# hanyujin02/trajectory_planner

Hardware: AMD Instinct MI355X
Metric: B-spline trajs/s (32 ctrl pts, 256^3 grid, 50 iters) @1 GPU; % HBM roofline (higher is better)
Workload: dtype f64

## Files before the change

trajectory_planner_amd/csrc/vigo_solver.hip:

```cpp
#include <stdlib.h>

#include <type_traits>

#include "vigo_internal.hpp"

namespace vigo {
namespace {

constexpr int kWave = 64;
constexpr int kMaxMem = VIGO_MAX_MEM_SIZE;
constexpr int kObsTabObs = 16;
template <int GROUP> constexpr int kObsTabEntries = GROUP == 32 ? 88 : 33;
template <int GROUP> constexpr int kObsTabDoubles = 3 * kObsTabEntries<GROUP> + kObsTabObs;

enum : int {
    LB_CONVERGENCE = 0,
    LB_STOP = 1,
    LB_ALREADY_MINIMIZED = 2,
    LBERR_UNKNOWN = -1024,
    LBERR_LOGIC,
    LBERR_CANCELED,
    LBERR_INVALID_N,
    LBERR_INVALID_MEMSIZE,
    LBERR_INVALID_GEPSILON,
// ... 56 lines not shown
__device__ __forceinline__ double dpp_f64(double v) {
    const int lo = __builtin_amdgcn_mov_dpp(__double2loint(v), CTRL, 0xF, 0xF, false);
    const int hi = __builtin_amdgcn_mov_dpp(__double2hiint(v), CTRL, 0xF, 0xF, false);
    return __hiloint2double(hi, lo);
}
__device__ __forceinline__ double add_f64_again(double a, double b) {
    double r;
    asm volatile("v_add_f64 %0, %1, %2" : "=v"(r) : "v"(a), "v"(b));
    return r;
}
__device__ __forceinline__ void xor16_parts(double a, double b, double& p0, double& p1) {
    const int alo = __double2loint(a), ahi = __double2hiint(a), blo = __double2loint(b), bhi = __double2hiint(b);
    auto l = __builtin_amdgcn_permlane16_swap(alo, blo, false, false);
    auto h = __builtin_amdgcn_permlane16_swap(ahi, bhi, false, false);
    p0 = __hiloint2double(h[0], l[0]);
    p1 = __hiloint2double(h[1], l[1]);
}
__device__ __forceinline__ double xor32_sum2(double a, double b) {
    const int alo = __double2loint(a), ahi = __double2hiint(a), blo = __double2loint(b), bhi = __double2hiint(b);
    auto l = __builtin_amdgcn_permlane32_swap(alo, blo, false, false);
    auto h = __builtin_amdgcn_permlane32_swap(ahi, bhi, false, false);
    return __hiloint2double(h[0], l[0]) + __hiloint2double(h[1], l[1]);
}
template <int GROUP, int K>
__device__ __forceinline__ void group_sum(double (&v)[K]) {
    static_assert(GROUP == 16 || GROUP == 32 || GROUP == 64, "group is a DPP row, half a wave or a wave");
#pragma unroll
    for (int q = 0; q < K; ++q) v[q] += dpp_f64<0xB1>(v[q]);
#pragma unroll
    for (int q = 0; q < K; ++q) v[q] += dpp_f64<0x4E>(v[q]);
#pragma unroll
    for (int q = 0; q < K; ++q) v[q] += dpp_f64<0x141>(v[q]);
    if (GROUP >= 32) {
#pragma unroll
        for (int q = 0; q < K; ++q) {
            const double t = dpp_f64<0x140>(v[q]);
            const double a = v[q] + t;
            const double b = add_f64_again(v[q], t);
            double p0, p1;
            xor16_parts(a, b, p0, p1);
            if (GROUP == 64) v[q] = xor32_sum2(p0 + p1, add_f64_again(p0, p1));
            else v[q] = p0 + p1;
        }
        return;
    }
#pragma unroll
// ... 29 lines not shown
        auto l2 = __builtin_amdgcn_permlane32_swap(xlo, xlo, false, false);
        auto h2 = __builtin_amdgcn_permlane32_swap(xhi, xhi, false, false);
        mx = fmax(__hiloint2double(h2[0], l2[0]), __hiloint2double(h2[1], l2[1]));
    }
}

__device__ __forceinline__ double sum3(double a, double b, double c) { return (a + b) + c; }

__device__ __forceinline__ double fmaT(double a, double b, double c) { return __builtin_fma(a, b, c); }
__device__ __forceinline__ float fmaT(float a, float b, float c) { return __builtin_fmaf(a, b, c); }

template <bool FAST, typename T, int D = 3>
__device__ __forceinline__ double dot3(const T (&a)[3], const T (&b)[3]) {
    if (D == 2) {
        if (FAST) return fmaT((double)a[1], (double)b[1], (double)a[0] * (double)b[0]);
        return (double)a[0] * (double)b[0] + (double)a[1] * (double)b[1];
    }
    if (FAST)
        return fmaT((double)a[2], (double)b[2], fmaT((double)a[1], (double)b[1], (double)a[0] * (double)b[0]));
    return sum3((double)a[0] * (double)b[0], (double)a[1] * (double)b[1], (double)a[2] * (double)b[2]);
}
template <bool FAST, typename T, int PPL, int D = 3>
__device__ __forceinline__ double dot_lane(const T (&a)[PPL][3], const T (&b)[PPL][3]) {
    double s = dot3<FAST, T, D>(a[0], b[0]);
#pragma unroll
    for (int q = 1; q < PPL; ++q) s += dot3<FAST, T, D>(a[q], b[q]);
    return s;
}

template <bool FAST>
struct YSv {
    double v, r;
};
template <>
struct YSv<true> {
    double v;
};
__device__ __forceinline__ bool exp_in_safe_range(double a) {
    const unsigned e = ((unsigned)__double2hiint(a) >> 20) & 0x7ffu;
    return (e - 523u) < 1000u;
}
__device__ __forceinline__ YSv<true> make_ys(double ys, YSv<true>*) { return YSv<true>{1.0 / ys}; }
__device__ __forceinline__ YSv<false> make_ys(double ys, YSv<false>*) {
    return YSv<false>{ys, exp_in_safe_range(ys) ? 1.0 / ys : __builtin_nan("")};
}
template <bool MARK>
__device__ __forceinline__ double over_ys(double a, const YSv<true>& y, double&, double&) { return a * y.v; }
template <bool MARK>
__device__ __forceinline__ double over_ys(double a, const YSv<false>& y, double& amin, double& amax) {
    if (!MARK) return a / y.v;
// ... 12 lines not shown

template <typename T, int PPL>
struct LaneProblem {
    static constexpr int kGuideRegs = (PPL == 1) ? 2 : 0;
    static constexpr int kGuideDim = kGuideRegs > 0 ? kGuideRegs : 1;
    int N;
    bool level;
    int p0;
    bool has_pt[PPL];
    bool interior[PPL];
    int g_begin[PPL], g_end[PPL];
    const double* gpv;
    const uint8_t* gunk;
    T gq[kGuideDim][6];
    bool gqu[kGuideDim];
    int o_begin, o_end;
    const double* obs;
    const double* obs_tab;
    const double* obs_size;
    int o_tab, o_steps;
    double w[4];
};

template <bool FAST, typename T>
__device__ __forceinline__ void guide_pair_term(const DevConst& K, const T (&c)[3], T px, T py, T pz, T vx,
                                                T vy, T vz, bool unk, double& cd, T (&Gd)[3]) {
    const T dth = (T)K.dth, da = (T)K.da, db = (T)K.db, dcc = (T)K.dc, uf = (T)K.unc_factor;
    const T dist = FAST ? fmaT(c[2] - pz, vz, fmaT(c[1] - py, vy, (c[0] - px) * vx))
                        : ((c[0] - px) * vx + (c[1] - py) * vy) + (c[2] - pz) * vz;
    const T e = dth - dist;
    T ct, k;
    bool scale = false;
    if (e <= -dth) {
        const T ne = -e;
        ct = (ne * ne) * ne;
        k = T(3.0) * (ne * ne);
    } else if (e > T(0) && e <= dth) {
        ct = (e * e) * e;
        k = T(-3.0) * (e * e);
        scale = unk;
    } else if (e >= dth) {
        ct = (da * (e * e) + db * e) + dcc;
        k = -((T(2) * da) * e + db);
        scale = unk;
    } else {
        return;
    }
    T gx = k * vx, gy = k * vy, gz = k * vz;
    if (scale) { ct *= uf; gx *= uf; gy *= uf; gz *= uf; }
    if (!K.plan_in_z) gz = T(0.0);
    cd += (double)ct;
    Gd[0] += gx; Gd[1] += gy; Gd[2] += gz;
}

template <typename T>
__device__ __forceinline__ void obstacle_term(const DevConst& K, const T (&c)[3], T opx, T opy, T ovx, T ovy, T size,
                                              double& co, T (&Go)[3]) {
    const T thr0 = (T)K.thr_dyn, oa = (T)K.oa, ob = (T)K.ob, oc = (T)K.oc;
    for (int n = 0; n <= K.pred_num; n += 2) {
        const T tn = (T)((double)n * K.ts);
        const T px = opx + tn * ovx, py = opy + tn * ovy;
        const T thr = (T(1) - (T)(n / K.pred_num) * T(0.2)) * thr0;
        const T dx = c[0] - px, dy = c[1] - py, dz = T(0.0);
        const T nrm = sqrt((dx * dx + dy * dy) + dz * dz);
        const T e = thr - (nrm - size);
        if (e > T(0)) {
            const bool cubic = e <= thr;
            const T ct = cubic ? (e * e) * e : (oa * (e * e) + ob * e) + oc;
            const T k = cubic ? T(-3.0) * (e * e) : -((T(2) * oa) * e + ob);
            co += (double)ct;
            Go[0] += k * (dx / nrm); Go[1] += k * (dy / nrm);
            if (__builtin_expect(!(nrm > T(0) && nrm < (T)INFINITY), 0)) Go[2] += k * (dz / nrm);
        }
    }
}

template <typename T>
__device__ __forceinline__ void obstacle_term_tab(const DevConst& K, const T (&c)[3], const double* tab, int steps,
                                                  T size, double& co, T (&Go)[3]) {
    const T oa = (T)K.oa, ob = (T)K.ob, oc = (T)K.oc;
    for (int s = 0; s < steps; ++s) {
        const T px = (T)tab[3 * s + 0], py = (T)tab[3 * s + 1], thr = (T)tab[3 * s + 2];
        const T dx = c[0] - px, dy = c[1] - py, dz = T(0.0);
        const T nrm = sqrt((dx * dx + dy * dy) + dz * dz);
        const T e = thr - (nrm - size);
        if (e > T(0)) {
            const bool cubic = e <= thr;
            const T ct = cubic ? (e * e) * e : (oa * (e * e) + ob * e) + oc;
            const T k = cubic ? T(-3.0) * (e * e) : -((T(2) * oa) * e + ob);
            co += (double)ct;
            Go[0] += k * (dx / nrm); Go[1] += k * (dy / nrm);
            if (__builtin_expect(!(nrm > T(0) && nrm < (T)INFINITY), 0)) Go[2] += k * (dz / nrm);
        }
    }
}

template <typename T, int GROUP, int PPL, bool FAST, bool OBS = true, int D = 3>
__device__ __forceinline__ double eval_cost_grad(const DevConst& K, const LaneProblem<T, PPL>& Q,
                                                 const T (&c)[PPL][3], const T (&d)[PPL][3], T (&g)[PPL][3],
                                                 double (&sums)[7]) {
    using LP = LaneProblem<T, PPL>;
    const int N = Q.N;
    T Gd[PPL][3], Gs[PPL][3], Gf[PPL][3], Go[PPL][3];
    double pt_s[PPL], pt_f[PPL], pt_d[PPL], pt_o[PPL];
#pragma unroll
    for (int q = 0; q < PPL; ++q) {
        pt_s[q] = pt_f[q] = pt_d[q] = pt_o[q] = 0.0;
#pragma unroll
        for (int a = 0; a < 3; ++a) Gd[q][a] = Go[q][a] = T(0);
    }

    {
        const T ts = (T)K.ts_ctrl, tis = (T)K.ts_inv_sqr;
        auto excess = [](T v) -> T { return v > T(1.0) ? v - T(1.0) : (v < T(-1.0) ? v + T(1.0) : T(0.0)); };
        double jj[PPL][3], vv[PPL][3], aa[PPL][3];
#pragma unroll
        for (int a = 0; a < 3; ++a) {
            if (a >= D) {
#pragma unroll
                for (int q = 0; q < PPL; ++q) { jj[q][a] = vv[q][a] = aa[q][a] = 0.0; Gs[q][a] = Gf[q][a] = T(0); }
                continue;
            }
            T C[PPL], P1[PPL], P2[PPL], P3[PPL];
#pragma unroll
            for (int q = 0; q < PPL; ++q) C[q] = c[q][a];
            seq_next<T, PPL>(C, P1);
            seq_next<T, PPL>(P1, P2);
            seq_next<T, PPL>(P2, P3);
            T gt0[PPL], gv[PPL], ga[PPL];
#pragma unroll
            for (int q = 0; q < PPL; ++q) {
                T J0 = FAST ? fmaT(T(3), P1[q], fmaT(T(-3), P2[q], P3[q])) - C[q]
                            : ((P3[q] - 3 * P2[q]) + 3 * P1[q]) - C[q];
                if (a == 2 && Q.level) J0 = T(0);
                gt0[q] = T(2.0) * J0;
                jj[q][a] = (double)(J0 * J0);
                T evP = excess((P1[q] - C[q]) / ts);
                T eaP = excess((FAST ? fmaT(T(-2), P1[q], P2[q]) + C[q]
                                     : (P2[q] - 2 * P1[q]) + C[q]) * tis);
                if (a == 2 && Q.level) { evP = T(0); eaP = T(0); }
                gv[q] = (T(2) * evP) / ts * tis;
                ga[q] = (T(2) * eaP) * tis;
                vv[q][a] = (double)((evP * evP) * tis);
                aa[q][a] = (double)(eaP * eaP);
            }
            T gt1[PPL], gt2[PPL], gt3[PPL], gvM[PPL], gaM1[PPL], gaM2[PPL];
            seq_prev<T, PPL>(gt0, gt1);
            seq_prev<T, PPL>(gt1, gt2);
            seq_prev<T, PPL>(gt2, gt3);
            seq_prev<T, PPL>(gv, gvM);
            seq_prev<T, PPL>(ga, gaM1);
            seq_prev<T, PPL>(gaM1, gaM2);
#pragma unroll
            for (int q = 0; q < PPL; ++q) {
                T acc = gt3[q];
                if (FAST) {
                    acc = fmaT(T(-3.0), gt2[q], acc);
                    acc = fmaT(T(3.0), gt1[q], acc);
                } else {
                    acc += T(-3.0) * gt2[q];
                    acc += T(3.0) * gt1[q];
                }
                acc += -gt0[q];
                Gs[q][a] = acc;
                T fcc = gvM[q];
                fcc += -gv[q];
                fcc += gaM2[q];
                fcc += -(T(2) * gaM1[q]);
                fcc += ga[q];
                Gf[q][a] = fcc;
            }
        }
#pragma unroll
        for (int q = 0; q < PPL; ++q) {
            const int p = Q.p0 + q;
            if (Q.has_pt[q] && p <= N - 4) pt_s[q] = sum3(jj[q][0], jj[q][1], jj[q][2]);
            double cf = 0.0;
            if (Q.has_pt[q] && p <= N - 2) cf = (vv[q][0] + vv[q][1]) + vv[q][2];
            if (Q.has_pt[q] && p <= N - 3) { cf += aa[q][0]; cf += aa[q][1]; cf += aa[q][2]; }
            pt_f[q] = cf;
        }
    }

#pragma unroll
    for (int q = 0; q < PPL; ++q) {
        if (Q.interior[q]) {
            double cd = 0.0;
            const int cnt = Q.g_end[q] - Q.g_begin[q];
#pragma unroll
            for (int j = 0; j < LP::kGuideRegs; ++j) {
                if (j < cnt)
                    guide_pair_term<FAST, T>(K, c[q], Q.gq[j][0], Q.gq[j][1], Q.gq[j][2], Q.gq[j][3], Q.gq[j][4], Q.gq[j][5],
                                       Q.gqu[j], cd, Gd[q]);
            }
// ... 56 lines not shown
        const double v4 = dot3<FAST, T, D>(g[q], d[q]);
        const double v5 = Q.interior[q] ? dot3<FAST, T>(c[q], c[q]) : 0.0;
        const double v6 = dot3<FAST, T, D>(g[q], g[q]);
        if (q == 0) {
            part[0] = pt_d[0]; part[1] = pt_s[0]; part[2] = pt_f[0]; part[3] = pt_o[0];
            part[4] = v4; part[5] = v5; part[6] = v6;
        } else {
            part[0] += pt_d[q]; part[1] += pt_s[q]; part[2] += pt_f[q]; part[3] += pt_o[q];
            part[4] += v4; part[5] += v5; part[6] += v6;
        }
    }
    if (OBS) {
        group_sum<GROUP, 7>(part);
    } else {
        double p6[6] = {part[0], part[1], part[2], part[4], part[5], part[6]};
        group_sum<GROUP, 6>(p6);
        part[0] = p6[0]; part[1] = p6[1]; part[2] = p6[2]; part[3] = 0.0; part[4] = p6[3]; part[5] = p6[4]; part[6] = p6[5];
    }
#pragma unroll
    for (int q = 0; q < 7; ++q) sums[q] = part[q];
    return ((Q.w[0] * part[0] + Q.w[1] * part[1]) + Q.w[2] * part[2]) + Q.w[3] * part[3];
}

template <typename T, int GROUP, int PPL>
__device__ __forceinline__ void load_problem(const SolveArgs& A, const DevConst& K, int b, int lane_in_group,
                                             LaneProblem<T, PPL>& Q) {
    using LP = LaneProblem<T, PPL>;
    const int N = A.N;
    Q.N = N;
    Q.level = false;
    Q.p0 = lane_in_group * PPL;
    Q.gpv = A.guide_pv;
    Q.gunk = A.guide_unk;
#pragma unroll
    for (int q = 0; q < PPL; ++q) {
        const int p = Q.p0 + q;
        Q.has_pt[q] = p < N;
        Q.interior[q] = (p >= 3) && (p <= N - 4);
        Q.g_begin[q] = Q.g_end[q] = 0;
        if (Q.interior[q] && A.guide_off && A.guide_pv) {
            Q.g_begin[q] = A.guide_off[(size_t)b * N + p];
            Q.g_end[q] = A.guide_off[(size_t)b * N + p + 1];
        }
    }
#pragma unroll
    for (int j = 0; j < LP::kGuideDim; ++j) {
// ... 40 lines not shown
    }
}

template <typename T, int GROUP, int PPL>
__device__ __forceinline__ void set_level(const DevConst& K, LaneProblem<T, PPL>& Q, const T (&x)[PPL][3]) {
    double mn = INFINITY, mx = -INFINITY;
#pragma unroll
    for (int q = 0; q < PPL; ++q) {
        if (Q.has_pt[q]) { mn = fmin(mn, (double)x[q][2]); mx = fmax(mx, (double)x[q][2]); }
    }
    group_minmax<GROUP>(mn, mx);
    Q.level = !K.plan_in_z && !K.strict_z && (mx - mn) <= 0x1p-40 * fmax(1.0, fmax(fabs(mn), fabs(mx)));
}

template <typename T, int PPL>
__device__ __forceinline__ void store_points(const SolveArgs& A, int b, const LaneProblem<T, PPL>& Q, const T (&x)[PPL][3]) {
#pragma unroll
    for (int q = 0; q < PPL; ++q) {
        if (Q.has_pt[q]) {
            double* dst = A.ctrl + ((size_t)b * A.N + Q.p0 + q) * 3;
            dst[0] = (double)x[q][0]; dst[1] = (double)x[q][1]; dst[2] = (double)x[q][2];
        }
    }
}

template <typename T, int GROUP, int PPL, bool FAST>
__global__ void __launch_bounds__(kWave) k_cost_grad(SolveArgs A, const DevConst* __restrict__ Kp) {
    const DevConst& K = *Kp;
    constexpr int TPB = kWave / GROUP;
    const int lane = threadIdx.x;
    const int b = blockIdx.x * TPB + lane / GROUP;
    if (b >= A.B) return;
    LaneProblem<T, PPL> Q;
    load_problem<T, GROUP, PPL>(A, K, b, lane % GROUP, Q);
    T c[PPL][3], g[PPL][3], zero[PPL][3];
    load_points<T, PPL>(A, b, Q, c);
    set_level<T, GROUP, PPL>(K, Q, c);
#pragma unroll
    for (int q = 0; q < PPL; ++q) zero[q][0] = zero[q][1] = zero[q][2] = T(0);
    double sums[7];
    const double f = eval_cost_grad<T, GROUP, PPL, FAST>(K, Q, c, zero, g, sums);
#pragma unroll
    for (int q = 0; q < PPL; ++q) {
        if (Q.interior[q] && A.out_grad) {
            double* dst = A.out_grad + ((size_t)b * (A.N - 6) + (Q.p0 + q - 3)) * 3;
            dst[0] = (double)g[q][0]; dst[1] = (double)g[q][1]; dst[2] = (double)g[q][2];
// ... 109 lines not shown
    tt = newt;
    return 0;
}

#ifndef VIGO_PROFILE_SECTIONS
#define VIGO_PROFILE_SECTIONS 0
#endif
#if VIGO_PROFILE_SECTIONS
#define VIGO_TICK(acc)                                                   \
    do {                                                                 \
        __builtin_amdgcn_sched_barrier(0);                               \
        const long long now_ = (long long)__builtin_readcyclecounter();  \
        __builtin_amdgcn_sched_barrier(0);                               \
        acc += (double)(now_ - tick_);                                   \
        tick_ = now_;                                                    \
    } while (0)
#else
#define VIGO_TICK(acc) do { } while (0)
#endif

template <typename T, int GROUP, int PPL, bool FAST, int WPS = 1, bool OBS = true, int D = 3, int RH = (PPL == 1 ? 1 : 0)>
__global__ void __launch_bounds__(kWave, WPS) k_optimize(SolveArgs A, const DevConst* __restrict__ Kp) {
    static_assert(PPL == 1 ? (RH >= 1 && RH <= 6) : RH == 0, "register-held history only with one point per lane");
    const DevConst& K = *Kp;
    constexpr int TPB = kWave / GROUP;
    extern __shared__ __align__(16) unsigned char lds_raw[];
    const int N = A.N, NI = N - 6;
    const int ROW = TPB * NI;
    const int ROWP = ROW + 1;
    using YS = YSv<FAST>;
    constexpr int kYsSlotBytes = (TPB * (int)sizeof(YS) + 15) & ~15;
    const int slotB = ROWP * (int)sizeof(HPair<T, D>) + kYsSlotBytes;
    const int m = K.mem_size;
    constexpr bool REG1 = (PPL == 1);
    const int ms = REG1 ? (m > RH + 1 ? m - (RH + 1) : 0) : m;
    HPair<T, D>* hist = reinterpret_cast<HPair<T, D>*>(lds_raw);
    double* ys_tab = reinterpret_cast<double*>(lds_raw + (size_t)ms * slotB);

    const int lane = threadIdx.x;
    const int grp = lane / GROUP;
    int b = blockIdx.x * TPB + grp;
    if (A.active_idx) {
        if (b >= *A.active_count) return;
        b = A.active_idx[b];
    } else if (b >= A.B) {
        return;
    }

    LaneProblem<T, PPL> Q;
    load_problem<T, GROUP, PPL>(A, K, b, lane % GROUP, Q);
    T x[PPL][3];
    load_points<T, PPL>(A, b, Q, x);
    set_level<T, GROUP, PPL>(K, Q, x);
    {
        const bool wave_level = __all(Q.level);
        if (D == 2 && !wave_level) return;
        if (D == 3 && A.level_waves_elsewhere && wave_level) return;
    }
#if VIGO_PROFILE_SECTIONS
    long long tick_ = (long long)__builtin_readcyclecounter();
    double t_eval = 0, t_ls = 0, t_upd = 0, t_two = 0, t_tail = 0, t_pre = 0, t_trial = 0, t_cal = 0;
#endif
    HPair<T, D>* hl[PPL];
#pragma unroll
    for (int q = 0; q < PPL; ++q) {
        const int p = Q.p0 + q;
        hl[q] = Q.interior[q] ? hist + (grp * NI + (p - 3)) : hist + ROW;
    }
    for (int slot = lane; slot < ms; slot += kWave) {
        HPair<T, D> zero;
#pragma unroll
        for (int a = 0; a < D; ++a) zero.s[a] = zero.y[a] = T(0);
        *reinterpret_cast<HPair<T, D>*>(lds_raw + (size_t)slot * slotB + (size_t)ROW * sizeof(HPair<T, D>)) = zero;
    }
    __syncthreads();
    YS* ys_l = reinterpret_cast<YS*>(lds_raw + (size_t)ROWP * sizeof(HPair<T, D>)) + grp;
    double* al_l = ys_tab + grp;
    auto hist_at = [&](int q, int slot) -> HPair<T, D>& {
        return *reinterpret_cast<HPair<T, D>*>(reinterpret_cast<char*>(hl[q]) + (size_t)slot * slotB);
    };
    auto ys_at = [&](int slot) -> YS& { return *reinterpret_cast<YS*>(reinterpret_cast<char*>(ys_l) + (size_t)slot * slotB); };
    if (!OBS) { Q.obs = nullptr; Q.o_begin = Q.o_end = 0; }
    if (OBS && A.obs) {
        constexpr int kEnt = kObsTabEntries<GROUP>;
        double* tab = ys_tab + (size_t)m * TPB + (size_t)grp * kObsTabDoubles<GROUP>;
        const int cnt = Q.o_end - Q.o_begin;
        const int steps = K.pred_num / 2 + 1;
        int fit = kEnt / steps;
        if (fit > kObsTabObs) fit = kObsTabObs;
        Q.o_tab = cnt < fit ? cnt : fit;
        Q.o_steps = steps;
        Q.obs_tab = tab;
        Q.obs_size = tab + 3 * kEnt;
        for (int e = lane % GROUP; e < Q.o_tab * steps; e += GROUP) {
            const int j = e / steps, n = 2 * (e - j * steps);
            const double* o = A.obs + 9 * (size_t)(Q.o_begin + j);
            const T tn = (T)((double)n * K.ts);
            tab[3 * e + 0] = (double)((T)o[0] + tn * (T)o[3]);
            tab[3 * e + 1] = (double)((T)o[1] + tn * (T)o[4]);
            tab[3 * e + 2] = (double)((T(1) - (T)(n / K.pred_num) * T(0.2)) * (T)K.thr_dyn);
        }
        for (int j = lane % GROUP; j < Q.o_tab; j += GROUP) {
            const double* o = A.obs + 9 * (size_t)(Q.o_begin + j);
            const T hx = (T)o[6] / 2, hy = (T)o[7] / 2;
            tab[3 * kEnt + j] = (double)(T)sqrt(hx * hx + hy * hy);
        }
        __syncthreads();
    }

    T g[PPL][3], xp[PPL][3], gp[PPL][3], d[PPL][3];
#pragma unroll
    for (int q = 0; q < PPL; ++q)
#pragma unroll
        for (int a = 0; a < 3; ++a) g[q][a] = xp[q][a] = gp[q][a] = d[q][a] = T(0);
    constexpr int kRH = RH > 0 ? RH : 1;
    T sR[kRH][PPL][3], yR[kRH][PPL][3];
    YS ysR[kRH]{};
#pragma unroll
    for (int q = 0; q < PPL; ++q)
#pragma unroll
        for (int a = 0; a < 3; ++a)
#pragma unroll
            for (int j = 0; j < kRH; ++j) sR[j][q][a] = yR[j][q][a] = T(0);
    double sums[7];
    int evals = 0;
    int ret = LBERR_UNKNOWN;
    int k = 0, end = 0, last = 0;
    double fx = 0.0, step = 0.0;
    bool first = true;

    for (;;) {
        int ls = 0;
        int count = 0, brackt = 0, stage1 = 1, uinfo = 0;
        double dginit = 0.0, finit = 0.0, dgtest = 0.0, width = 0.0, prev_width = 0.0;
        double xt = 0., xf = 0., xd = 0., yt = 0., yf = 0., yd = 0.;
        const double stpmin = K.min_step, stpmax = K.max_step;
        bool run = true;
        if (!first) {
#pragma unroll
            for (int q = 0; q < PPL; ++q)
#pragma unroll
                for (int a = 0; a < D; ++a) { xp[q][a] = x[q][a]; gp[q][a] = g[q][a]; }
            dginit = sums[4];
            if (step <= 0.) { ls = LBERR_INVALIDPARAMETERS; run = false; }
            else if (0 < dginit) { ls = LBERR_INCREASEGRADIENT; run = false; }
            finit = fx;
            dgtest = K.ftol * dginit;
            width = stpmax - stpmin;
            prev_width = 2.0 * width;
            xt = yt = 0.;
            xf = yf = finit;
            xd = yd = dginit;
        }
        while (run) {
            double stmin = 0., stmax = 0.;
            if (!first) {
                if (brackt) {
                    stmin = xt <= yt ? xt : yt;
                    stmax = xt >= yt ? xt : yt;
                } else {
                    stmin = xt;
                    stmax = step + 4.0 * (step - xt);
                }
                if (step < stpmin) step = stpmin;
                if (stpmax < step) step = stpmax;
                if ((brackt && ((step <= stmin || stmax <= step) || K.max_linesearch <= count + 1 || uinfo != 0)) ||
                    (brackt && (stmax - stmin <= K.xtol * stmax))) {
                    step = xt;
                }
#pragma unroll
                for (int q = 0; q < PPL; ++q)
#pragma unroll
                    for (int a = 0; a < D; ++a)
                        x[q][a] = FAST ? fmaT((T)step, d[q][a], xp[q][a]) : xp[q][a] + (T)step * d[q][a];
            }

            VIGO_TICK(t_pre);
            fx = eval_cost_grad<T, GROUP, PPL, FAST, OBS, D>(K, Q, x, d, g, sums);
            VIGO_TICK(t_eval);
            ++evals;
            if (first) break;

            const double dg = sums[4];
            const double ftest1 = finit + step * dgtest;
            ++count;

            {
                int code = 0;
                if (fx <= ftest1 && fabs(dg) <= K.gtol * (-dginit)) code = count;
                if (K.max_linesearch <= count) code = LBERR_MAXIMUMLINESEARCH;
                if (brackt && (stmax - stmin) <= K.xtol * stmax) code = LBERR_WIDTHTOOSMALL;
                if (step == stpmin && (ftest1 < fx || dgtest <= dg)) code = LBERR_MINIMUMSTEP;
                if (step == stpmax && fx <= ftest1 && dg <= dgtest) code = LBERR_MAXIMUMSTEP;
                if (brackt && ((step <= stmin || stmax <= step) || uinfo != 0)) code = LBERR_ROUNDING_ERROR;
                if (code != 0) { ls = code; break; }
            }

            const double cmin = K.ftol <= K.gtol ? K.ftol : K.gtol;
            if (stage1 && fx <= ftest1 && cmin * dginit <= dg) stage1 = 0;

            const bool mod = stage1 && ftest1 < fx && fx <= xf;
// ... 13 lines not shown
                prev_width = width;
                width = fabs(yt - xt);
            }
        }

        VIGO_TICK(t_ls);
        double xnorm = sqrt(sums[5]), gnorm = sqrt(sums[6]);
        if (first) {
            first = false;
#pragma unroll
            for (int q = 0; q < PPL; ++q)
#pragma unroll
                for (int a = 0; a < D; ++a) d[q][a] = -g[q][a];
            if (xnorm < 1.0) xnorm = 1.0;
            if (gnorm / xnorm <= K.g_epsilon) { ret = LB_ALREADY_MINIMIZED; break; }
            step = 1.0 / sqrt(sums[6]);
            sums[4] = -sums[6];
            k = 1;
            end = 0;
            continue;
        }

        if (ls < 0) {
            store_points<T, PPL>(A, b, Q, x);
#pragma unroll
            for (int q = 0; q < PPL; ++q)
#pragma unroll
                for (int a = 0; a < D; ++a) { x[q][a] = xp[q][a]; g[q][a] = gp[q][a]; }
            ret = ls;
            break;
        }

        if (xnorm < 1.0) xnorm = 1.0;
        if (gnorm / xnorm <= K.g_epsilon) { ret = LB_CONVERGENCE; break; }
        if (K.max_iterations != 0 && K.max_iterations < k + 1) { ret = LBERR_MAXIMUMITERATION; break; }

        T sv[PPL][3], yv[PPL][3];
#pragma unroll
        for (int q = 0; q < PPL; ++q) {
#pragma unroll
            for (int a = 0; a < D; ++a) { sv[q][a] = x[q][a] - xp[q][a]; yv[q][a] = g[q][a] - gp[q][a]; }
            if (!REG1 && Q.interior[q]) {
                HPair<T, D> hp;
#pragma unroll
                for (int a = 0; a < D; ++a) { hp.s[a] = sv[q][a]; hp.y[a] = yv[q][a]; }
                hist_at(q, end) = hp;
            }
        }
        double ysyy[2] = {dot_lane<FAST, T, PPL, D>(yv, sv), dot_lane<FAST, T, PPL, D>(yv, yv)};
        if (D == 2) ysyy[0] += 0.0;
        group_sum<GROUP, 2>(ysyy);
        const double ys = ysyy[0], yy = ysyy[1];
        const YS ys_div = make_ys(ys, static_cast<YS*>(nullptr));
        if (!REG1) ys_at(end) = ys_div;
        const bool haveR = REG1 && k >= RH + 1;

        const int bound = (m <= k) ? m : k;
        const int newest = REG1 ? last : end;
        if (!REG1) end = (end + 1 == m) ? 0 : end + 1;
        ++k;
#pragma unroll
        for (int q = 0; q < PPL; ++q)
#pragma unroll
            for (int a = 0; a < D; ++a) d[q][a] = -g[q][a];

        constexpr int kWin = 2;
        T Ps[kWin][PPL][3], Py[kWin][PPL][3];
        YS Pys[kWin];
        auto fetch = [&](int age, T (&s_)[PPL][3], T (&y_)[PPL][3], YS& ys_) {
            if (REG1 && age == 0) {
#pragma unroll
                for (int q = 0; q < PPL; ++q)
#pragma unroll
// ... 117 lines not shown
                }
            }
            if (!MARK) return false;
            bool bad = !(amin >= 0x1p-500) || !(amax <= 0x1p500);
#pragma unroll
            for (int q = 0; q < PPL; ++q)
#pragma unroll
                for (int a = 0; a < D; ++a) bad |= !(d[q][a] == d[q][a]);
            return bad;
        };
        VIGO_TICK(t_upd);
        if (PPL == 1 && bound == kMaxMem && !__any(last != __builtin_amdgcn_readfirstlane(last))) {
            if (__any(two_loop(std::true_type{}))) {
                asm volatile("" ::: "memory");
#pragma unroll
                for (int q = 0; q < PPL; ++q)
#pragma unroll
                    for (int a = 0; a < D; ++a) d[q][a] = -g[q][a];
                two_loop(std::false_type{});
            }
        } else {
            two_loop(std::false_type{});
        }
#pragma unroll
        for (int q = 0; q < PPL; ++q)
#pragma unroll
            for (int a = 0; a < D; ++a) d[q][a] = Q.interior[q] ? d[q][a] : T(0);
        VIGO_TICK(t_two);
        if (REG1) {
            if (haveR && ms > 0) {
#pragma unroll
                for (int q = 0; q < PPL; ++q) {
                    if (Q.interior[q]) {
                        HPair<T, D> hp;
#pragma unroll
                        for (int a = 0; a < D; ++a) { hp.s[a] = sR[kRH - 1][q][a]; hp.y[a] = yR[kRH - 1][q][a]; }
                        hist_at(q, end) = hp;
                    }
                }
                ys_at(end) = ysR[kRH - 1];
                last = end;
                end = (end + 1 == ms) ? 0 : end + 1;
            }
#pragma unroll
            for (int j = kRH - 1; j > 0; --j) {
#pragma unroll
                for (int q = 0; q < PPL; ++q)
#pragma unroll
                    for (int a = 0; a < D; ++a) { sR[j][q][a] = sR[j - 1][q][a]; yR[j][q][a] = yR[j - 1][q][a]; }
                ysR[j] = ysR[j - 1];
            }
#pragma unroll
            for (int q = 0; q < PPL; ++q)
#pragma unroll
                for (int a = 0; a < D; ++a) { sR[0][q][a] = sv[q][a]; yR[0][q][a] = yv[q][a]; }
            ysR[0] = ys_div;
        }
        sums[4] = group_sum1<GROUP>(dot_lane<FAST, T, PPL, D>(g, d));
        step = 1.0;
        VIGO_TICK(t_tail);
        VIGO_TICK(t_cal);
    }

    if (ret >= 0 || ret == LBERR_MAXIMUMITERATION) store_points<T, PPL>(A, b, Q, x);
#pragma unroll
    for (int q = 0; q < PPL; ++q) {
        if (Q.interior[q] && A.out_x) {
            double* dst = A.out_x + ((size_t)b * NI + (Q.p0 + q - 3)) * 3;
            dst[0] = (double)x[q][0]; dst[1] = (double)x[q][1]; dst[2] = (double)x[q][2];
        }
    }
#if VIGO_PROFILE_SECTIONS
    if (lane % GROUP == 0 && A.out_x) {
        double* o = A.out_x + (size_t)b * NI * 3;
        o[0] = t_eval; o[1] = t_ls; o[2] = t_upd; o[3] = t_two; o[4] = t_tail; o[5] = (double)k; o[6] = (double)evals;
        o[7] = t_pre; o[8] = t_trial; o[9] = t_cal;
    }
#endif
    if (lane % GROUP == 0) {
        if (A.out_status) A.out_status[(size_t)b * (A.status_stride ? A.status_stride : 1)] = ret;
        if (A.out_fx) A.out_fx[b] = fx;
        if (A.out_iters) A.out_iters[b] = k;
        if (A.out_evals) A.out_evals[b] = evals;
    }
}

template <typename T, int GROUP, bool FAST, int D = 3>
size_t optimize_lds_bytes(int N, int m, int ppl, bool with_obstacles, int rh = 1) {
    const int TPB = kWave / GROUP;
    const int ms = ppl == 1 ? (m > rh + 1 ? m - (rh + 1) : 0) : m;
    const size_t slot = ((size_t)TPB * (N - 6) + 1) * sizeof(HPair<T, D>) + (((size_t)TPB * sizeof(YSv<FAST>) + 15) & ~(size_t)15);
    size_t h = (size_t)ms * slot;
    h += (size_t)m * TPB * sizeof(double);
    if (with_obstacles) h += (size_t)TPB * kObsTabDoubles<GROUP> * sizeof(double);
    return h;
}

constexpr size_t kLdsPerWorkgroup = 160 * 1024;

}

#ifndef VIGO_SOLVER_PART
#define VIGO_SOLVER_PART 0
#endif

#if VIGO_SOLVER_PART == 0
DevConst make_dev_const(const vigo_params_t& P) {
    DevConst K{};
    K.dth = P.dthresh;
    K.da = 3.0 * P.dthresh;
    K.db = -3.0 * pow(P.dthresh, 2);
    K.dc = pow(P.dthresh, 3);
    K.unc_factor = P.uncertain_factor;
    K.hth = 0.2;
// ... 44 lines not shown
    return (int)hipGetLastError();
}

int launch_cost_grad(hipStream_t s, const SolveArgs& a, const DevConst& k, const DevConst* kd, int precision) {
    (void)k;
    if (a.B <= 0) return hipSuccess;
    if (precision == VIGO_PREC_F32) return launch_cost_grad_t<float, false>(s, a, kd);
    if (precision == VIGO_PREC_F64_FAST) return launch_cost_grad_t<double, true>(s, a, kd);
    return launch_cost_grad_t<double, false>(s, a, kd);
}
#endif

template <typename KernelT>
static int raise_dynamic_lds(LaunchState& L, int slot, KernelT kernel) {
    if (L.lds_attr_set & (1ull << slot)) return (int)hipSuccess;
    hipError_t e = hipFuncSetAttribute(reinterpret_cast<const void*>(kernel), hipFuncAttributeMaxDynamicSharedMemorySize,
                                       (int)kLdsPerWorkgroup);
    if (e != hipSuccess) return (int)e;
    L.lds_attr_set |= 1ull << slot;
    return (int)hipSuccess;
}

constexpr int kLevelRH = 4, kLevelRH64 = 5;
template <typename T, int GROUP, int PPL, bool FAST, bool OBS>
static int launch_optimize_t(hipStream_t s, const SolveArgs& a_in, const DevConst& k, const DevConst* kd, LaunchState& L) {
    const int tpb = kWave / GROUP;
    SolveArgs a = a_in;
    dim3 grid((a.B + tpb - 1) / tpb), block(kWave);
    const int arith = std::is_same<T, float>::value ? 0 : (FAST ? 2 : 1);
    const int shape = GROUP == 32 ? 0 : (PPL == 1 ? 1 : (PPL == 2 ? 2 : 3));
    const int slot = (arith * 4 + shape) * 4;
    const int simds = L.simd_count > 0 ? L.simd_count : (1 << 30);
    auto go = [&](auto kernel, int sl, size_t lds) -> int {
        int e = raise_dynamic_lds(L, sl, kernel);
        if (e != (int)hipSuccess) return e;
        hipLaunchKernelGGL(kernel, grid, block, lds, s, a, kd);
        return (int)hipGetLastError();
    };
    constexpr bool kHasLevel = PPL == 1 && !OBS;
    const bool two = kHasLevel && !k.plan_in_z && !k.strict_z;
    a.level_waves_elsewhere = two ? 1 : 0;
    const size_t lds = optimize_lds_bytes<T, GROUP, FAST, 3>(a.N, k.mem_size, PPL, a.obs != nullptr);
    if (lds > kLdsPerWorkgroup) return (int)hipErrorInvalidValue;
    int e = (int)hipSuccess;
    if constexpr (kHasLevel) {
        if (two) {
            const size_t lds2 = optimize_lds_bytes<T, GROUP, FAST, 2>(a.N, k.mem_size, PPL, false);
            const int slot2 = 48 + arith * 4 + shape * 2;
            constexpr int kRH = GROUP == 32 ? kLevelRH : kLevelRH64;
            constexpr bool kHasRH = std::is_same<T, double>::value && kRH > 1;
            bool done = false;
            if constexpr (kHasRH) {
                const size_t lds3 = optimize_lds_bytes<T, GROUP, FAST, 2>(a.N, k.mem_size, PPL, false, kRH);
                if ((int)grid.x > simds && lds2 > kLdsPerWorkgroup / 8 && kLdsPerWorkgroup / lds3 > kLdsPerWorkgroup / lds2) {
                    constexpr int kWps = kRH >= 4 ? 2 : 1;
                    e = go(&k_optimize<T, GROUP, PPL, FAST, kWps, OBS, 2, kRH>, 60 + (FAST ? 1 : 0) + (GROUP == 64 ? 2 : 0), lds3);
                    done = true;
                }
            }
            if (!done) {
                if ((int)grid.x > simds && lds2 <= kLdsPerWorkgroup / 8) e = go(&k_optimize<T, GROUP, PPL, FAST, 2, OBS, 2>, slot2 + 1, lds2);
                else e = go(&k_optimize<T, GROUP, PPL, FAST, 1, OBS, 2>, slot2, lds2);
            }
            if (e != (int)hipSuccess) return e;
        }
    }
    if (PPL == 1 && (int)grid.x > simds && lds <= kLdsPerWorkgroup / 8) {
        if constexpr (PPL == 1) e = go(&k_optimize<T, GROUP, PPL, FAST, 2, OBS, 3>, slot + (OBS ? 1 : 3), lds);
        else e = (int)hipErrorInvalidValue;
    } else {
        e = go(&k_optimize<T, GROUP, PPL, FAST, 1, OBS, 3>, slot + (OBS ? 0 : 2), lds);
    }
    return e;
}

template <typename T, bool FAST, bool OBS>
static int launch_optimize_p(hipStream_t s, const SolveArgs& a, const DevConst& k, const DevConst* kd, LaunchState& L) {
    switch (shape_for(a.N)) {
        case 0: return launch_optimize_t<T, 32, 1, FAST, OBS>(s, a, k, kd, L);
        case 1: return launch_optimize_t<T, 64, 1, FAST, OBS>(s, a, k, kd, L);
        case 2: return launch_optimize_t<T, 64, 2, FAST, OBS>(s, a, k, kd, L);
// ... 36 lines not shown
```

Measured before the change: 3.378 million.

## Add axis-per-lane layout for level trajectories when batch fits SIMDs

```diff
diff --git a/trajectory_planner_amd/csrc/vigo_solver.hip b/trajectory_planner_amd/csrc/vigo_solver.hip
--- a/trajectory_planner_amd/csrc/vigo_solver.hip
+++ b/trajectory_planner_amd/csrc/vigo_solver.hip
@@ -102,6 +102,21 @@
     auto h = __builtin_amdgcn_permlane32_swap(ahi, bhi, false, false);
     return __hiloint2double(h[0], l[0]) + __hiloint2double(h[1], l[1]);
 }
+__device__ __forceinline__ void xy_parts(double a, double b, double& x, double& y) {
+    const int alo = __double2loint(a), ahi = __double2hiint(a), blo = __double2loint(b), bhi = __double2hiint(b);
+    auto l = __builtin_amdgcn_permlane32_swap(alo, blo, false, false);
+    auto h = __builtin_amdgcn_permlane32_swap(ahi, bhi, false, false);
+    x = __hiloint2double(h[0], l[0]);
+    y = __hiloint2double(h[1], l[1]);
+}
+__device__ __forceinline__ void xy_both(double v, double& x, double& y) { xy_parts(v, v, x, y); }
+__device__ __forceinline__ double mul_f64_again(double a, double b) {
+    double r;
+    asm volatile("v_mul_f64 %0, %1, %2" : "=v"(r) : "v"(a), "v"(b));
+    return r;
+}
+__device__ __forceinline__ double dot_xy(double a, double b) { return xor32_sum2(a * b, mul_f64_again(a, b)); }
+
 template <int GROUP, int K>
 __device__ __forceinline__ void group_sum(double (&v)[K]) {
     static_assert(GROUP == 16 || GROUP == 32 || GROUP == 64, "group is a DPP row, half a wave or a wave");
@@ -177,10 +192,15 @@
 }
 template <bool FAST, typename T, int PPL, int D = 3>
 __device__ __forceinline__ double dot_lane(const T (&a)[PPL][3], const T (&b)[PPL][3]) {
-    double s = dot3<FAST, T, D>(a[0], b[0]);
-#pragma unroll
-    for (int q = 1; q < PPL; ++q) s += dot3<FAST, T, D>(a[q], b[q]);
-    return s;
+    if constexpr (D == 1) {
+        static_assert(!FAST && PPL == 1, "the axis-per-lane layout is reference order, one point per lane pair");
+        return dot_xy((double)a[0][0], (double)b[0][0]);
+    } else {
+        double s = dot3<FAST, T, D>(a[0], b[0]);
+#pragma unroll
+        for (int q = 1; q < PPL; ++q) s += dot3<FAST, T, D>(a[q], b[q]);
+        return s;
+    }
 }
 
 template <bool FAST>
@@ -239,15 +259,11 @@
     double w[4];
 };
 
-template <bool FAST, typename T>
-__device__ __forceinline__ void guide_pair_term(const DevConst& K, const T (&c)[3], T px, T py, T pz, T vx,
-                                                T vy, T vz, bool unk, double& cd, T (&Gd)[3]) {
-    const T dth = (T)K.dth, da = (T)K.da, db = (T)K.db, dcc = (T)K.dc, uf = (T)K.unc_factor;
-    const T dist = FAST ? fmaT(c[2] - pz, vz, fmaT(c[1] - py, vy, (c[0] - px) * vx))
-                        : ((c[0] - px) * vx + (c[1] - py) * vy) + (c[2] - pz) * vz;
+template <typename T>
+__device__ __forceinline__ bool guide_penalty(const DevConst& K, T dist, bool unk, T& ct, T& k, bool& scale) {
+    const T dth = (T)K.dth, da = (T)K.da, db = (T)K.db, dcc = (T)K.dc;
     const T e = dth - dist;
-    T ct, k;
-    bool scale = false;
+    scale = false;
     if (e <= -dth) {
         const T ne = -e;
         ct = (ne * ne) * ne;
@@ -261,13 +277,36 @@
         k = -((T(2) * da) * e + db);
         scale = unk;
     } else {
-        return;
-    }
+        return false;
+    }
+    return true;
+}
+template <bool FAST, typename T>
+__device__ __forceinline__ void guide_pair_term(const DevConst& K, const T (&c)[3], T px, T py, T pz, T vx,
+                                                T vy, T vz, bool unk, double& cd, T (&Gd)[3]) {
+    const T uf = (T)K.unc_factor;
+    const T dist = FAST ? fmaT(c[2] - pz, vz, fmaT(c[1] - py, vy, (c[0] - px) * vx))
+                        : ((c[0] - px) * vx + (c[1] - py) * vy) + (c[2] - pz) * vz;
+    T ct, k;
+    bool scale;
+    if (!guide_penalty<T>(K, dist, unk, ct, k, scale)) return;
     T gx = k * vx, gy = k * vy, gz = k * vz;
     if (scale) { ct *= uf; gx *= uf; gy *= uf; gz *= uf; }
     if (!K.plan_in_z) gz = T(0.0);
     cd += (double)ct;
     Gd[0] += gx; Gd[1] += gy; Gd[2] += gz;
+}
+__device__ __forceinline__ void guide_pair_term_axis(const DevConst& K, double c, double cz, double p, double pz, double v,
+                                                     double vz, bool unk, double& cd, double& Gd) {
+    const double uf = K.unc_factor;
+    const double dist = dot_xy(c - p, v) + (cz - pz) * vz;
+    double ct, k;
+    bool scale;
+    if (!guide_penalty<double>(K, dist, unk, ct, k, scale)) return;
+    double gc = k * v;
+    if (scale) { ct *= uf; gc *= uf; }
+    cd += ct;
+    Gd += gc;
 }
 
 template <typename T>
@@ -312,6 +351,60 @@
     }
 }
 
+template <typename T, int PPL, bool FAST>
+__device__ __forceinline__ void stencil_axis(const DevConst& K, const T (&C)[PPL], bool no_terms, double (&jj)[PPL],
+                                             double (&vv)[PPL], double (&aa)[PPL], T (&Gs)[PPL], T (&Gf)[PPL]) {
+    const T ts = (T)K.ts_ctrl, tis = (T)K.ts_inv_sqr;
+    auto excess = [](T v) -> T { return v > T(1.0) ? v - T(1.0) : (v < T(-1.0) ? v + T(1.0) : T(0.0)); };
+    T P1[PPL], P2[PPL], P3[PPL];
+    seq_next<T, PPL>(C, P1);
+    seq_next<T, PPL>(P1, P2);
+    seq_next<T, PPL>(P2, P3);
+    T gt0[PPL], gv[PPL], ga[PPL];
+#pragma unroll
+    for (int q = 0; q < PPL; ++q) {
+        T J0 = FAST ? fmaT(T(3), P1[q], fmaT(T(-3), P2[q], P3[q])) - C[q]
+                    : ((P3[q] - 3 * P2[q]) + 3 * P1[q]) - C[q];
+        if (no_terms) J0 = T(0);
+        gt0[q] = T(2.0) * J0;
+        jj[q] = (double)(J0 * J0);
+        T evP = excess((P1[q] - C[q]) / ts);
+        T eaP = excess((FAST ? fmaT(T(-2), P1[q], P2[q]) + C[q]
+                             : (P2[q] - 2 * P1[q]) + C[q]) * tis);
+        if (no_terms) { evP = T(0); eaP = T(0); }
+        gv[q] = (T(2) * evP) / ts * tis;
+        ga[q] = (T(2) * eaP) * tis;
+        vv[q] = (double)((evP * evP) * tis);
+        aa[q] = (double)(eaP * eaP);
+    }
+    T gt1[PPL], gt2[PPL], gt3[PPL], gvM[PPL], gaM1[PPL], gaM2[PPL];
+    seq_prev<T, PPL>(gt0, gt1);
+    seq_prev<T, PPL>(gt1, gt2);
+    seq_prev<T, PPL>(gt2, gt3);
+    seq_prev<T, PPL>(gv, gvM);
+    seq_prev<T, PPL>(ga, gaM1);
+    seq_prev<T, PPL>(gaM1, gaM2);
+#pragma unroll
+    for (int q = 0; q < PPL; ++q) {
+        T acc = gt3[q];
+        if (FAST) {
+            acc = fmaT(T(-3.0), gt2[q], acc);
+            acc = fmaT(T(3.0), gt1[q], acc);
+        } else {
+            acc += T(-3.0) * gt2[q];
+            acc += T(3.0) * gt1[q];
+        }
+        acc += -gt0[q];
+        Gs[q] = acc;
+        T fcc = gvM[q];
+        fcc += -gv[q];
+        fcc += gaM2[q];
+        fcc += -(T(2) * gaM1[q]);
+        fcc += ga[q];
+        Gf[q] = fcc;
+    }
+}
+
 template <typename T, int GROUP, int PPL, bool FAST, bool OBS = true, int D = 3>
 __device__ __forceinline__ double eval_cost_grad(const DevConst& K, const LaneProblem<T, PPL>& Q,
                                                  const T (&c)[PPL][3], const T (&d)[PPL][3], T (&g)[PPL][3],
@@ -328,8 +421,6 @@
     }
 
     {
-        const T ts = (T)K.ts_ctrl, tis = (T)K.ts_inv_sqr;
-        auto excess = [](T v) -> T { return v > T(1.0) ? v - T(1.0) : (v < T(-1.0) ? v + T(1.0) : T(0.0)); };
         double jj[PPL][3], vv[PPL][3], aa[PPL][3];
 #pragma unroll
         for (int a = 0; a < 3; ++a) {
@@ -338,55 +429,13 @@
                 for (int q = 0; q < PPL; ++q) { jj[q][a] = vv[q][a] = aa[q][a] = 0.0; Gs[q][a] = Gf[q][a] = T(0); }
                 continue;
             }
-            T C[PPL], P1[PPL], P2[PPL], P3[PPL];
+            T C[PPL], GsA[PPL], GfA[PPL];
+            double jjA[PPL], vvA[PPL], aaA[PPL];
 #pragma unroll
             for (int q = 0; q < PPL; ++q) C[q] = c[q][a];
-            seq_next<T, PPL>(C, P1);
-            seq_next<T, PPL>(P1, P2);
-            seq_next<T, PPL>(P2, P3);
-            T gt0[PPL], gv[PPL], ga[PPL];
-#pragma unroll
-            for (int q = 0; q < PPL; ++q) {
-                T J0 = FAST ? fmaT(T(3), P1[q], fmaT(T(-3), P2[q], P3[q])) - C[q]
-                            : ((P3[q] - 3 * P2[q]) + 3 * P1[q]) - C[q];
-                if (a == 2 && Q.level) J0 = T(0);
-                gt0[q] = T(2.0) * J0;
-                jj[q][a] = (double)(J0 * J0);
-                T evP = excess((P1[q] - C[q]) / ts);
-                T eaP = excess((FAST ? fmaT(T(-2), P1[q], P2[q]) + C[q]
-                                     : (P2[q] - 2 * P1[q]) + C[q]) * tis);
-                if (a == 2 && Q.level) { evP = T(0); eaP = T(0); }
-                gv[q] = (T(2) * evP) / ts * tis;
-                ga[q] = (T(2) * eaP) * tis;
-                vv[q][a] = (double)((evP * evP) * tis);
-                aa[q][a] = (double)(eaP * eaP);
-            }
-            T gt1[PPL], gt2[PPL], gt3[PPL], gvM[PPL], gaM1[PPL], gaM2[PPL];
-            seq_prev<T, PPL>(gt0, gt1);
-            seq_prev<T, PPL>(gt1, gt2);
-            seq_prev<T, PPL>(gt2, gt3);
-            seq_prev<T, PPL>(gv, gvM);
-            seq_prev<T, PPL>(ga, gaM1);
-            seq_prev<T, PPL>(gaM1, gaM2);
-#pragma unroll
-            for (int q = 0; q < PPL; ++q) {
-                T acc = gt3[q];
-                if (FAST) {
-                    acc = fmaT(T(-3.0), gt2[q], acc);
-                    acc = fmaT(T(3.0), gt1[q], acc);
-                } else {
-                    acc += T(-3.0) * gt2[q];
-                    acc += T(3.0) * gt1[q];
-                }
-                acc += -gt0[q];
-                Gs[q][a] = acc;
-                T fcc = gvM[q];
-                fcc += -gv[q];
-                fcc += gaM2[q];
-                fcc += -(T(2) * gaM1[q]);
-                fcc += ga[q];
-                Gf[q][a] = fcc;
-            }
+            stencil_axis<T, PPL, FAST>(K, C, a == 2 && Q.level, jjA, vvA, aaA, GsA, GfA);
+#pragma unroll
+            for (int q = 0; q < PPL; ++q) { jj[q][a] = jjA[q]; vv[q][a] = vvA[q]; aa[q][a] = aaA[q]; Gs[q][a] = GsA[q]; Gf[q][a] = GfA[q]; }
         }
 #pragma unroll
         for (int q = 0; q < PPL; ++q) {
@@ -489,6 +538,62 @@
     return ((Q.w[0] * part[0] + Q.w[1] * part[1]) + Q.w[2] * part[2]) + Q.w[3] * part[3];
 }
 
+__device__ __forceinline__ double eval_cost_grad_axis(const DevConst& K, const LaneProblem<double, 1>& Q, int axis,
+                                                      const double (&c)[1][3], const double (&d)[1][3], double (&g)[1][3],
+                                                      double (&sums)[7]) {
+    using LP = LaneProblem<double, 1>;
+    const int N = Q.N, p = Q.p0;
+    const double C[1] = {c[0][0]};
+    const double cz = c[0][2];
+    double jj[1], vv[1], aa[1], Gs[1], Gf[1];
+    stencil_axis<double, 1, false>(K, C, false, jj, vv, aa, Gs, Gf);
+    double j0, j1, v0, v1, a0, a1;
+    xy_both(jj[0], j0, j1);
+    xy_both(vv[0], v0, v1);
+    xy_both(aa[0], a0, a1);
+    double pt_s = 0.0, pt_f = 0.0, pt_d = 0.0;
+    if (Q.has_pt[0] && p <= N - 4) pt_s = sum3(j0, j1, 0.0);
+    if (Q.has_pt[0] && p <= N - 2) pt_f = (v0 + v1) + 0.0;
+    if (Q.has_pt[0] && p <= N - 3) { pt_f += a0; pt_f += a1; pt_f += 0.0; }
+
+    double Gd = 0.0;
+    if (Q.interior[0]) {
+        double cd = 0.0;
+        const int cnt = Q.g_end[0] - Q.g_begin[0];
+#pragma unroll
+        for (int j = 0; j < LP::kGuideRegs; ++j) {
+            if (j < cnt) guide_pair_term_axis(K, C[0], cz, Q.gq[j][0], Q.gq[j][2], Q.gq[j][3], Q.gq[j][5], Q.gqu[j], cd, Gd);
+        }
+        for (int j = Q.g_begin[0] + LP::kGuideRegs; j < Q.g_end[0]; ++j) {
+            const double* pv = Q.gpv + 6 * (size_t)j;
+            guide_pair_term_axis(K, C[0], cz, pv[axis], pv[2], pv[3 + axis], pv[5], Q.gunk ? (Q.gunk[j] != 0) : false, cd, Gd);
+        }
+        pt_d = cd;
+    }
+
+    const double w0 = Q.w[0], w1 = Q.w[1], w2 = Q.w[2], w3 = Q.w[3];
+    const double Go = 0.0;
+    g[0][0] = !Q.interior[0] ? 0.0 : ((w0 * Gd + w1 * Gs[0]) + w2 * Gf[0]) + w3 * Go;
+    g[0][1] = g[0][2] = 0.0;
+    double p6[6];
+    p6[0] = pt_d; p6[1] = pt_s; p6[2] = pt_f;
+    p6[3] = dot_xy(g[0][0], d[0][0]);
+    const double xx = dot_xy(C[0], C[0]) + cz * cz;
+    p6[4] = Q.interior[0] ? xx : 0.0;
+    p6[5] = dot_xy(g[0][0], g[0][0]);
+    group_sum<32, 6>(p6);
+    sums[0] = p6[0]; sums[1] = p6[1]; sums[2] = p6[2]; sums[3] = 0.0; sums[4] = p6[3]; sums[5] = p6[4]; sums[6] = p6[5];
+    return ((Q.w[0] * sums[0] + Q.w[1] * sums[1]) + Q.w[2] * sums[2]) + Q.w[3] * sums[3];
+}
+
+__device__ __forceinline__ void axis_guides(LaneProblem<double, 1>& Q, int axis) {
+#pragma unroll
+    for (int j = 0; j < LaneProblem<double, 1>::kGuideDim; ++j) {
+        Q.gq[j][0] = axis ? Q.gq[j][1] : Q.gq[j][0];
+        Q.gq[j][3] = axis ? Q.gq[j][4] : Q.gq[j][3];
+    }
+}
+
 template <typename T, int GROUP, int PPL>
 __device__ __forceinline__ void load_problem(const SolveArgs& A, const DevConst& K, int b, int lane_in_group,
                                              LaneProblem<T, PPL>& Q) {
@@ -575,6 +680,13 @@
             dst[0] = (double)x[q][0]; dst[1] = (double)x[q][1]; dst[2] = (double)x[q][2];
         }
     }
+}
+
+__device__ __forceinline__ void store_point_axis(const SolveArgs& A, int b, const LaneProblem<double, 1>& Q, int axis, double v, double z) {
+    if (!Q.has_pt[0]) return;
+    double* dst = A.ctrl + ((size_t)b * A.N + Q.p0) * 3;
+    dst[axis] = v;
+    if (axis == 0) dst[2] = z;
 }
 
 template <typename T, int GROUP, int PPL, bool FAST>
@@ -730,11 +842,15 @@
 template <typename T, int GROUP, int PPL, bool FAST, int WPS = 1, bool OBS = true, int D = 3, int RH = (PPL == 1 ? 1 : 0)>
 __global__ void __launch_bounds__(kWave, WPS) k_optimize(SolveArgs A, const DevConst* __restrict__ Kp) {
     static_assert(PPL == 1 ? (RH >= 1 && RH <= 6) : RH == 0, "register-held history only with one point per lane");
+    constexpr bool AXIS = D == 1;
+    static_assert(!AXIS || (std::is_same<T, double>::value && GROUP == 32 && PPL == 1 && !FAST && !OBS),
+                  "the axis-per-lane layout: fp64 reference order, N <= 32, no obstacles");
     const DevConst& K = *Kp;
-    constexpr int TPB = kWave / GROUP;
+    constexpr int TPB = AXIS ? 1 : kWave / GROUP;
+    constexpr int COLS = kWave / GROUP;
     extern __shared__ __align__(16) unsigned char lds_raw[];
     const int N = A.N, NI = N - 6;
-    const int ROW = TPB * NI;
+    const int ROW = COLS * NI;
     const int ROWP = ROW + 1;
     using YS = YSv<FAST>;
     constexpr int kYsSlotBytes = (TPB * (int)sizeof(YS) + 15) & ~15;
@@ -747,7 +863,8 @@
 
     const int lane = threadIdx.x;
     const int grp = lane / GROUP;
-    int b = blockIdx.x * TPB + grp;
+    const int tg = AXIS ? 0 : grp;
+    int b = blockIdx.x * TPB + tg;
     if (A.active_idx) {
         if (b >= *A.active_count) return;
         b = A.active_idx[b];
@@ -760,11 +877,16 @@
     T x[PPL][3];
     load_points<T, PPL>(A, b, Q, x);
     set_level<T, GROUP, PPL>(K, Q, x);
-    {
+    if constexpr (AXIS) {
+        if (!Q.level) return;
+        x[0][0] = grp ? x[0][1] : x[0][0];
+        axis_guides(Q, grp);
+    } else {
         const bool wave_level = __all(Q.level);
         if (D == 2 && !wave_level) return;
         if (D == 3 && A.level_waves_elsewhere && wave_level) return;
     }
+    const bool solved_elsewhere = D == 3 && A.level_waves_elsewhere == 2 && Q.level;
 #if VIGO_PROFILE_SECTIONS
     long long tick_ = (long long)__builtin_readcyclecounter();
     double t_eval = 0, t_ls = 0, t_upd = 0, t_two = 0, t_tail = 0, t_pre = 0, t_trial = 0, t_cal = 0;
@@ -782,8 +904,9 @@
         *reinterpret_cast<HPair<T, D>*>(lds_raw + (size_t)slot * slotB + (size_t)ROW * sizeof(HPair<T, D>)) = zero;
     }
     __syncthreads();
-    YS* ys_l = reinterpret_cast<YS*>(lds_raw + (size_t)ROWP * sizeof(HPair<T, D>)) + grp;
-    double* al_l = ys_tab + grp;
+    if (solved_elsewhere) return;
+    YS* ys_l = reinterpret_cast<YS*>(lds_raw + (size_t)ROWP * sizeof(HPair<T, D>)) + tg;
+    double* al_l = ys_tab + tg;
     auto hist_at = [&](int q, int slot) -> HPair<T, D>& {
         return *reinterpret_cast<HPair<T, D>*>(reinterpret_cast<char*>(hl[q]) + (size_t)slot * slotB);
     };
@@ -830,6 +953,7 @@
         for (int a = 0; a < 3; ++a)
 #pragma unroll
             for (int j = 0; j < kRH; ++j) sR[j][q][a] = yR[j][q][a] = T(0);
+    T dz = T(-0.0);
     double sums[7];
     int evals = 0;
     int ret = LBERR_UNKNOWN;
@@ -849,6 +973,7 @@
             for (int q = 0; q < PPL; ++q)
 #pragma unroll
                 for (int a = 0; a < D; ++a) { xp[q][a] = x[q][a]; gp[q][a] = g[q][a]; }
+            if constexpr (AXIS) xp[0][2] = x[0][2];
             dginit = sums[4];
             if (step <= 0.) { ls = LBERR_INVALIDPARAMETERS; run = false; }
             else if (0 < dginit) { ls = LBERR_INCREASEGRADIENT; run = false; }
@@ -881,10 +1006,12 @@
 #pragma unroll
                     for (int a = 0; a < D; ++a)
                         x[q][a] = FAST ? fmaT((T)step, d[q][a], xp[q][a]) : xp[q][a] + (T)step * d[q][a];
+                if constexpr (AXIS) x[0][2] = xp[0][2] + (T)step * (Q.interior[0] ? dz : T(0));
             }
 
             VIGO_TICK(t_pre);
-            fx = eval_cost_grad<T, GROUP, PPL, FAST, OBS, D>(K, Q, x, d, g, sums);
+            if constexpr (AXIS) fx = eval_cost_grad_axis(K, Q, grp, x, d, g, sums);
+            else fx = eval_cost_grad<T, GROUP, PPL, FAST, OBS, D>(K, Q, x, d, g, sums);
             VIGO_TICK(t_eval);
             ++evals;
             if (first) break;
@@ -944,11 +1071,13 @@
         }
 
         if (ls < 0) {
-            store_points<T, PPL>(A, b, Q, x);
+            if constexpr (AXIS) store_point_axis(A, b, Q, grp, x[0][0], x[0][2]);
+            else store_points<T, PPL>(A, b, Q, x);
 #pragma unroll
             for (int q = 0; q < PPL; ++q)
 #pragma unroll
                 for (int a = 0; a < D; ++a) { x[q][a] = xp[q][a]; g[q][a] = gp[q][a]; }
+            if constexpr (AXIS) x[0][2] = xp[0][2];
             ret = ls;
             break;
         }
@@ -970,7 +1099,7 @@
             }
         }
         double ysyy[2] = {dot_lane<FAST, T, PPL, D>(yv, sv), dot_lane<FAST, T, PPL, D>(yv, yv)};
-        if (D == 2) ysyy[0] += 0.0;
+        if (D <= 2) ysyy[0] += 0.0;
         group_sum<GROUP, 2>(ysyy);
         const double ys = ysyy[0], yy = ysyy[1];
         const YS ys_div = make_ys(ys, static_cast<YS*>(nullptr));
@@ -1134,6 +1263,9 @@
         } else {
             two_loop(std::false_type{});
         }
+        if constexpr (AXIS)
+            dz = __hiloint2double(__builtin_amdgcn_readfirstlane(__double2hiint(d[0][0])),
+                                  __builtin_amdgcn_readfirstlane(__double2loint(d[0][0])));
 #pragma unroll
         for (int q = 0; q < PPL; ++q)
 #pragma unroll
@@ -1174,12 +1306,20 @@
         VIGO_TICK(t_cal);
     }
 
-    if (ret >= 0 || ret == LBERR_MAXIMUMITERATION) store_points<T, PPL>(A, b, Q, x);
+    if (ret >= 0 || ret == LBERR_MAXIMUMITERATION) {
+        if constexpr (AXIS) store_point_axis(A, b, Q, grp, x[0][0], x[0][2]);
+        else store_points<T, PPL>(A, b, Q, x);
+    }
 #pragma unroll
     for (int q = 0; q < PPL; ++q) {
         if (Q.interior[q] && A.out_x) {
             double* dst = A.out_x + ((size_t)b * NI + (Q.p0 + q - 3)) * 3;
-            dst[0] = (double)x[q][0]; dst[1] = (double)x[q][1]; dst[2] = (double)x[q][2];
+            if constexpr (AXIS) {
+                dst[grp] = (double)x[q][0];
+                if (grp == 0) dst[2] = (double)x[q][2];
+            } else {
+                dst[0] = (double)x[q][0]; dst[1] = (double)x[q][1]; dst[2] = (double)x[q][2];
+            }
         }
     }
 #if VIGO_PROFILE_SECTIONS
@@ -1189,7 +1329,7 @@
         o[7] = t_pre; o[8] = t_trial; o[9] = t_cal;
     }
 #endif
-    if (lane % GROUP == 0) {
+    if (lane % (kWave / TPB) == 0) {
         if (A.out_status) A.out_status[(size_t)b * (A.status_stride ? A.status_stride : 1)] = ret;
         if (A.out_fx) A.out_fx[b] = fx;
         if (A.out_iters) A.out_iters[b] = k;
@@ -1199,9 +1339,10 @@
 
 template <typename T, int GROUP, bool FAST, int D = 3>
 size_t optimize_lds_bytes(int N, int m, int ppl, bool with_obstacles, int rh = 1) {
-    const int TPB = kWave / GROUP;
+    const int TPB = D == 1 ? 1 : kWave / GROUP;
+    const int COLS = kWave / GROUP;
     const int ms = ppl == 1 ? (m > rh + 1 ? m - (rh + 1) : 0) : m;
-    const size_t slot = ((size_t)TPB * (N - 6) + 1) * sizeof(HPair<T, D>) + (((size_t)TPB * sizeof(YSv<FAST>) + 15) & ~(size_t)15);
+    const size_t slot = ((size_t)COLS * (N - 6) + 1) * sizeof(HPair<T, D>) + (((size_t)TPB * sizeof(YSv<FAST>) + 15) & ~(size_t)15);
     size_t h = (size_t)ms * slot;
     h += (size_t)m * TPB * sizeof(double);
     if (with_obstacles) h += (size_t)TPB * kObsTabDoubles<GROUP> * sizeof(double);
@@ -1292,6 +1433,17 @@
 }
 
 constexpr int kLevelRH = 4, kLevelRH64 = 5;
+#ifndef VIGO_EXP_AXIS_SWITCH
+#define VIGO_EXP_AXIS_SWITCH 0
+#endif
+static inline bool axis_dispatch_on() {
+#if VIGO_EXP_AXIS_SWITCH
+    const char* e = getenv("VIGO_EXP_AXIS");
+    return !(e && e[0] == '0');
+#else
+    return true;
+#endif
+}
 template <typename T, int GROUP, int PPL, bool FAST, bool OBS>
 static int launch_optimize_t(hipStream_t s, const SolveArgs& a_in, const DevConst& k, const DevConst* kd, LaunchState& L) {
     const int tpb = kWave / GROUP;
@@ -1320,13 +1472,24 @@
             constexpr int kRH = GROUP == 32 ? kLevelRH : kLevelRH64;
             constexpr bool kHasRH = std::is_same<T, double>::value && kRH > 1;
             bool done = false;
+            if constexpr (std::is_same<T, double>::value && !FAST && GROUP == 32) {
+                if (L.simd_count > 0 && a.B <= L.simd_count && axis_dispatch_on()) {
+                    const size_t lds1 = optimize_lds_bytes<T, GROUP, FAST, 1>(a.N, k.mem_size, PPL, false);
+                    hipLaunchKernelGGL((k_optimize<T, GROUP, PPL, FAST, 1, OBS, 1>), dim3(a.B), block, lds1, s, a, kd);
+                    e = (int)hipGetLastError();
+                    a.level_waves_elsewhere = 2;
+                    done = true;
+                }
+            }
             if constexpr (kHasRH) {
+              if (!done) {
                 const size_t lds3 = optimize_lds_bytes<T, GROUP, FAST, 2>(a.N, k.mem_size, PPL, false, kRH);
                 if ((int)grid.x > simds && lds2 > kLdsPerWorkgroup / 8 && kLdsPerWorkgroup / lds3 > kLdsPerWorkgroup / lds2) {
                     constexpr int kWps = kRH >= 4 ? 2 : 1;
                     e = go(&k_optimize<T, GROUP, PPL, FAST, kWps, OBS, 2, kRH>, 60 + (FAST ? 1 : 0) + (GROUP == 64 ? 2 : 0), lds3);
                     done = true;
                 }
+              }
             }
             if (!done) {
                 if ((int)grid.x > simds && lds2 <= kLdsPerWorkgroup / 8) e = go(&k_optimize<T, GROUP, PPL, FAST, 2, OBS, 2>, slot2 + 1, lds2);
```

After: 3.486 million (median of 6 runs). 3.2% higher.
